# BurnhamG/PyTorch-ScalableFHVAE

Hardware: AMD Instinct MI355X
Metric: segments/sec + ELBO (nats/frame), (B,20,80) fbank (higher is better)
Workload: dtype bf16

## Files before the change

### include/fhvae_hip.h

```cpp
#ifndef FHVAE_HIP_H
#define FHVAE_HIP_H

#include <stdint.h>

#ifdef __cplusplus
extern "C" {
#endif

#define FHVAE_ABI_VERSION 11

enum { FHVAE_F32 = 0, FHVAE_BF16 = 1 };

enum {
  FHVAE_OK = 0,
  FHVAE_ERR_NULL = -1,
  FHVAE_ERR_SHAPE = -2,
  FHVAE_ERR_DTYPE = -3,
  FHVAE_ERR_ALIGN = -4,
  FHVAE_ERR_LIMIT = -5
};

#define FHVAE_MAX_LAYERS 4
#define FHVAE_LSTM_SYNC_BYTES 16384

// ... 46 lines not shown
  const float* b_ih[FHVAE_MAX_LAYERS];
  const float* b_hh[FHVAE_MAX_LAYERS];
  void* hs;
  float* cs;
  void* gates;
  float* hn;
  float* hs_top_f32;
  float* pre;
  void* lp;
  void* hn_lp;
  const float* head_w_mu;
  const float* head_w_lv;
  void* head_wl;
  void* head_wt;
  int64_t head_D, head_K, head_ldt;
  int32_t* sticky_status;
} fhvae_lstm_desc;

int64_t fhvae_lstm_lp_bytes(const fhvae_lstm_desc* d);
int64_t fhvae_lstm_pre_elems(const fhvae_lstm_desc* d);
int fhvae_lstm_layout_id(const fhvae_lstm_desc* d);

int64_t fhvae_lstm_ws_below_elems(const fhvae_lstm_desc* d);
int fhvae_lstm_form(const fhvae_lstm_desc* d);
int fhvae_lstm_seq_fwd(const fhvae_lstm_desc* d, void* stream);

typedef struct fhvae_lstm_bwd_desc {
  fhvae_lstm_desc f;
  const float* d_hs_top;
  const float* d_hn;
  void* dgates;
  float* dgsum;
  float* dc;
  float* dw_ih[FHVAE_MAX_LAYERS];
  float* dw_hh[FHVAE_MAX_LAYERS];
  float* db_ih[FHVAE_MAX_LAYERS];
  float* db_hh[FHVAE_MAX_LAYERS];
  float* d_xc;
  int32_t phase;
  float* ws_below;
} fhvae_lstm_bwd_desc;

int fhvae_lstm_seq_bwd(const fhvae_lstm_bwd_desc* d, void* stream);
typedef struct fhvae_wgrad_desc {
  const void* a; int64_t lda;
  int64_t a_col0;
  const void* b; int64_t ldb;
  float* c; int64_t ldc;
  int64_t M, N, K;
} fhvae_wgrad_desc;
int fhvae_wgrad_desc_ok(const fhvae_wgrad_desc* p);
int fhvae_lstm_param_grads_multi(const fhvae_lstm_bwd_desc* const* descs, int n, const fhvae_wgrad_desc* extra, int n_extra,
                                 void* stream);
int fhvae_wgrad_bf16(const void* a, int64_t lda, const void* b, int64_t ldb, float* c, int64_t ldc, int64_t M,
                     int64_t N, int64_t K, void* stream);
int fhvae_wgrad_f32(const float* a, int64_t lda, const float* b, int64_t ldb, float* c, int64_t ldc, int64_t M, int64_t N,
                    int64_t K, void* stream);

int fhvae_proj_bf16(const void* a, int64_t lda, const void* b, int64_t ldb, const float* bias, float* c, int64_t ldc,
                    int64_t M, int64_t N, int64_t K, void* stream);

int fhvae_mu2_gather_fwd(const float* table, const int64_t* idx, int64_t idx_offset, float* mu2,
                         int64_t B, int64_t S, int64_t D, int32_t* oob_flag, void* stream);
int fhvae_mu2_gather_bwd(const float* dmu2, const int64_t* idx, int64_t idx_offset, float* dtable,
                         int64_t B, int64_t S, int64_t D, float scale, void* stream);

typedef struct fhvae_elbo_desc {
  int64_t B, T, F, D1, D2;
  const float* x;    int64_t x_sb, x_st;
  const float* x_mu; const float* x_lv; int64_t xo_sb, xo_st;
  const float* z1_mu; const float* z1_lv;
  const float* z2_mu; const float* z2_lv;
  const float* mu2;
  const int64_t* num_segs; double nsegs_scalar;
  float* lower_bound; float* log_px_z; float* neg_kld_z1; float* neg_kld_z2; float* log_pmu2;
} fhvae_elbo_desc;

int fhvae_elbo_fwd(const fhvae_elbo_desc* d, void* stream);

typedef struct fhvae_elbo_bwd_desc {
  fhvae_elbo_desc f;
  const float* g_lower_bound; const float* g_log_px_z; const float* g_neg_kld_z1;
  const float* g_neg_kld_z2; const float* g_log_pmu2;
  int32_t reference_detach;
  float* d_x_mu; float* d_x_lv;
  float* d_z1_mu; float* d_z1_lv; float* d_z2_mu; float* d_z2_lv; float* d_mu2;
  void* d_x_pair_lp; int64_t ld_pair; float* d_x_colsum;
} fhvae_elbo_bwd_desc;

int fhvae_elbo_bwd(const fhvae_elbo_bwd_desc* d, void* stream);
int64_t fhvae_elbo_colsum_rows(int64_t B);

int64_t fhvae_disc_lse_ws_bytes(int64_t B, int64_t S);
int fhvae_disc_lse_fwd(const float* q, const float* table, const int64_t* idx, int64_t row0,
                       float inv_two_var, float* row_max, float* row_sumexp, float* tgt_logit,
                       float* ce_mean, float ce_scale, void* ws, int64_t B, int64_t S, int64_t D, int dtype, void* stream);
int fhvae_shard_pack(const float* q, const int64_t* idx, float* out, int64_t B, int64_t D, void* stream);
int fhvae_shard_unpack(const float* packed, float* q, int64_t* idx, int64_t N, int64_t D, void* stream);
int fhvae_disc_merge_partials(const float* parts, float* row_max, float* row_sumexp, float* tgt_logit, int64_t W, int64_t N,
                              void* stream);
int fhvae_shard_bwd_pack(const float* dq_all, float dq_scale, const float* dmu2_local, int64_t own0, int64_t n_own, float* out,
                         int64_t N, int64_t D, void* stream);
int fhvae_shard_bwd_unpack(const float* buf, int64_t own0, int64_t n_own, float* dq_local, float* dmu2_all, int64_t N, int64_t D,
                           void* stream);
int fhvae_disc_ce_mean(const float* row_max, const float* row_sumexp, const float* tgt_logit,
                       float* ce_mean, float ce_scale, int64_t B, void* stream);
// ... 40 lines not shown
```

### pytorch-scalablefhvae_amd/csrc/lstm.hip

```cpp
#include "gemm_launch.h"
#include "lstm_cell.h"
#include "lstm_cluster.h"
#include "wgrad.h"
#include "wgrad_f32.h"
#include <algorithm>
#include <vector>
#include "trace.h"
#include <cstdlib>

namespace fh {

constexpr int kCH = 32;

struct GateRowMap {
  int H;
  __device__ __forceinline__ int64_t operator()(int n) const {
    int unit = (n >> 6) * 16 + (n & 15);
    int gate = (n & 63) >> 4;
    return unit < H ? (int64_t)gate * H + unit : -1;
  }
  __device__ __forceinline__ bool all_valid(int n0, int n) const { return ((n0 + n) >> 6) * 16 <= H; }
};

template <typename T>
// ... 693 lines not shown
  if constexpr (!kF32) {
    if (cluster_eligible(d)) {
      ClusterWeights cw = {};
      for (int l = 0; l < L; ++l) cw.w_ih[l] = op.w_ih[l], cw.w_hh[l] = op.w_hh[l], cw.w_ih_t[l] = op.w_ih_t[l], cw.w_hh_t[l] = op.w_hh_t[l];
      cw.xch = (u16*)d->lp + lp_layout(d).xch;
      return cluster_bwd(bd, cw, st);
    }
  }
  if (big_cells(B, H, d->dtype) && cell_bwd_plan_ok(bd, op)) {
    for (int64_t w = 0; w < T_ + L - 1; ++w) {
      int nj = 0;
      const BwdJobs<T> jobs = bwd_jobs<T>(bd, op, w, nj);
      double fl = 0;
      for (int j = 0; j < nj; ++j) fl += 2.0 * B * H * (jobs.job[j].seg[0].K + jobs.job[j].seg[1].K);
      const int ts = trace_begin(st, kTraceBwdCell, fl);
      const int e = launch_cell_bwd_big(jobs, nj, st);
      trace_end(st, ts);
      if (e) return e;
    }
    if (Ic > 0) return launch_cell_dgsum((const T*)bd->dgates, bd->dgsum, (int)T_, B * 4 * H, st);
    return FHVAE_OK;
  }
  for (int64_t w = 0; w < T_ + L - 1; ++w) {
    int nj = 0;
    const BwdJobs<T> jobs = bwd_jobs<T>(bd, op, w, nj);
    double fl = 0;
    for (int j = 0; j < nj; ++j) fl += 2.0 * B * H * (jobs.job[j].seg[0].K + jobs.job[j].seg[1].K);
    const int ts = trace_begin(st, kTraceBwdCell, fl);
    const int bt = B >= 16384 ? 128 : 32;
    if (bt == 128) {
      dim3 grid((unsigned)fh_cdiv(B, 128), (unsigned)fh_cdiv(H, 64), (unsigned)nj);
      hipLaunchKernelGGL((lstm_bwd_step_kernel<T, 128, 64, 4, 1, 16>), grid, dim3(kThreads), 0, st, jobs);
    } else if (bt == 64) {
      dim3 grid((unsigned)fh_cdiv(B, 64), (unsigned)fh_cdiv(H, 64), (unsigned)nj);
      hipLaunchKernelGGL((lstm_bwd_step_kernel<T, 64, 64, 2, 2, 16>), grid, dim3(kThreads), 0, st, jobs);
    } else if (B >= 1024) {
      dim3 grid((unsigned)fh_cdiv(B, 32), (unsigned)fh_cdiv(H, 32), (unsigned)nj);
      hipLaunchKernelGGL((lstm_bwd_step_kernel<T, 32, 32, 2, 2, 16>), grid, dim3(kThreads), 0, st, jobs);
    } else {
      dim3 grid((unsigned)fh_cdiv(B, 32), (unsigned)fh_cdiv(H, 32), (unsigned)nj);
      hipLaunchKernelGGL((lstm_bwd_step_kernel<T, 32, 32, 2, 2, kCH>), grid, dim3(kThreads), 0, st, jobs);
    }
    trace_end(st, ts);
    int e = fh_launch_status();
    if (e) return e;
  }
  return FHVAE_OK;
}

constexpr int64_t kWgradMinK = 1024;

template <typename T>
static int lstm_param_grads(const fhvae_lstm_bwd_desc* bd, const Ops<T>& op, hipStream_t st, std::vector<WgProblem>* wq = nullptr,
                            std::vector<GemmParams>* fq = nullptr, std::vector<WgProblem32>* wq32 = nullptr) {
  const fhvae_lstm_desc* d = &bd->f;
  const int64_t B = d->B, T_ = d->T, I = d->I, Ic = d->Ic, H = d->H;
  const int L = d->L;
  const int64_t K0 = I + Ic, G = 4 * H;
  const T* dg = (const T*)bd->dgates;
  const T* hs = (const T*)d->hs;
  GemmParams grp[2 * FHVAE_MAX_LAYERS];
  int ng = 0;
  auto wgrad_long = [&](const void* a, int64_t lda, const void* b, int64_t ldb, int64_t Kc, float* c, int64_t ldc, int64_t Ncols) {
    if (sizeof(T) == 4) {
      if (!wq32 || Kc < kWgradMinK) return false;
      WgProblem32 w = {};
      w.A = (const float*)a, w.B = (const float*)b, w.C = c;
      w.lda = lda, w.ldb = ldb, w.ldc = ldc;
      w.M = (int)G, w.N = (int)Ncols, w.K = (int)Kc;
      if (!wgrad32_eligible(w)) return false;
      wq32->push_back(w);
      return true;
    }
    if (!wq || sizeof(T) != 2 || Kc < kWgradMinK) return false;
    WgProblem w = {};
    w.A = (const u16*)a, w.B = (const u16*)b, w.C = c;
    w.lda = lda, w.ldb = ldb, w.ldc = ldc;
    w.M = (int)G, w.N = (int)Ncols, w.K = (int)Kc;
    if (!wgrad_eligible(w)) return false;
    wq->push_back(w);
    return true;
  };
  auto wgrad = [&](const void* a, int64_t lda, const void* b, int64_t ldb, int64_t Kc, float* c, int64_t ldc, int64_t Ncols) {
    GemmParams p = {};
    p.seg[0] = Seg{a, lda, 0, b, ldb, 0, (int)Kc, 0};
    p.M = (int)G;
    p.N = (int)Ncols;
    p.C = c;
    p.ldc = ldc;
    p.splitk = 0;
    p.mode = 1;
    return p;
  };
  auto flush = [&]() -> int {
    int e = FHVAE_OK;
    for (int i = 0; i < ng && !e; i += kMaxGroup) e = launch_gemm_group(grp + i, ng - i < kMaxGroup ? ng - i : kMaxGroup, d->dtype, st);
    ng = 0;
    return e;
  };
  for (int l = 0; l < L; ++l) {
    const T* dgl = dg + (int64_t)l * T_ * B * G;
    const T* hl = hs + (int64_t)l * T_ * B * H;
    int e;
    if (bd->dw_hh[l] && T_ > 1 && !wgrad_long(dgl + B * G, G, hl, H, (T_ - 1) * B, bd->dw_hh[l], H, H))
      grp[ng++] = wgrad(dgl + B * G, G, hl, H, (T_ - 1) * B, bd->dw_hh[l], H, H);
    if (bd->dw_ih[l]) {
      if (l > 0) {
        if (!wgrad_long(dgl, G, hs + (int64_t)(l - 1) * T_ * B * H, H, T_ * B, bd->dw_ih[l], H, H))
          grp[ng++] = wgrad(dgl, G, hs + (int64_t)(l - 1) * T_ * B * H, H, T_ * B, bd->dw_ih[l], H, H);
      } else {
        if (I > 0 && !wgrad_long(dgl, G, op.x, I, T_ * B, bd->dw_ih[0], K0, I))
          grp[ng++] = wgrad(dgl, G, op.x, I, T_ * B, bd->dw_ih[0], K0, I);
        if (Ic > 0) {
          GemmParams p = wgrad(bd->dgsum, G, d->xc, Ic, B, bd->dw_ih[0] + I, K0, Ic);
          if (fq) {
            fq->push_back(p);
          } else {
            e = launch_gemm(p, FHVAE_F32, st);
            if (e) return e;
          }
        }
      }
    }
    if (!(sizeof(T) == 2 && cluster_eligible(d))) {
      if (l == 0 && Ic > 0 && bd->dgsum)
        e = launch_colsum(bd->dgsum, FHVAE_F32, G, bd->db_ih[l], bd->db_hh[l], B, G, st);
      else
        e = launch_colsum(dgl, d->dtype, G, bd->db_ih[l], bd->db_hh[l], T_ * B, G, st);
      if (e) return e;
    }
  }
  return flush();
}

static int lstm_dxc(const fhvae_lstm_bwd_desc* bd, hipStream_t st, bool zeroed = false) {
  const fhvae_lstm_desc* d = &bd->f;
  if (!bd->d_xc || d->Ic <= 0) return FHVAE_OK;
  const int64_t G = 4 * d->H, K0 = d->I + d->Ic;
  GemmParams p = {};
  p.seg[0] = Seg{bd->dgsum, G, 1, d->w_ih[0] + d->I, K0, 0, (int)G, 0};
  p.M = (int)d->B;
  p.N = (int)d->Ic;
  p.C = bd->d_xc;
  p.ldc = d->Ic;
  const int64_t tiles = fh_cdiv(d->B, 64) * fh_cdiv(d->Ic, 64);
  if (tiles <= 64 && G >= 512) {
    const int64_t n = d->B * d->Ic;
    if (!zeroed) hipLaunchKernelGGL(zero_f32_kernel, dim3((unsigned)fh_cdiv(n, 1024)), dim3(256), 0, st, bd->d_xc, n);
    p.mode = 2;
    int64_t sk = 256 / tiles;
    while (sk > 1 && G / sk < 128) sk >>= 1;
    p.splitk = (int)(sk < 4 ? 4 : sk > 16 ? 16 : sk);
  } else {
    p.splitk = 1;
  }
  return launch_gemm(p, FHVAE_F32, st);
}

extern "C" int fhvae_lstm_seq_bwd(const fhvae_lstm_bwd_desc* bd, void* stream) {
  FH_CHECK_PTR(bd);
  const fhvae_lstm_desc* d = &bd->f;
  int e = check_desc(d);
  if (e) return e;
  FH_CHECK_PTR(bd->dgates);
  FH_CHECK_PTR(bd->dc);
  if (d->Ic > 0) FH_CHECK_PTR(bd->dgsum);
  if (bd->phase < 0 || bd->phase > 2) return FHVAE_ERR_SHAPE;
  const bool rec = bd->phase != 2, par = bd->phase != 1;
  if (rec && !bd->d_hs_top && !bd->d_hn) return FHVAE_ERR_NULL;
  hipStream_t st = (hipStream_t)stream;
  if (d->dtype == FHVAE_F32) {
    Ops<float> op = ops_f32(d);
    if (rec) {
      e = lstm_bwd_impl<float>(bd, op, st);
      if (e) return e;
      e = lstm_dxc(bd, st);
      if (e) return e;
    }
    if (!par) return FHVAE_OK;
    std::vector<WgProblem32> wq32;
    e = lstm_param_grads<float>(bd, op, st, nullptr, nullptr, getenv("FHVAE_NO_WGRAD") ? nullptr : &wq32);
    if (e) return e;
    return launch_wgrad32(wq32.data(), (int)wq32.size(), st);
  }
  Ops<u16> op = ops_bf16(d);
  if (rec) {
    e = lstm_bwd_impl<u16>(bd, op, st);
    if (e) return e;
    e = lstm_dxc(bd, st, cluster_eligible(d) && cluster_bwd_zeroes_dxc(d));
    if (e) return e;
  }
  if (!par) return FHVAE_OK;
  std::vector<WgProblem> wq;
  e = lstm_param_grads<u16>(bd, op, st, getenv("FHVAE_NO_WGRAD") ? nullptr : &wq);
  if (e) return e;
  return launch_wgrad(wq.data(), (int)wq.size(), st);
}

static bool wg_from_desc(const fhvae_wgrad_desc* x, WgProblem& p) {
  if (!x || x->M <= 0 || x->N <= 0 || x->K <= 0 || x->M > INT32_MAX || x->N > INT32_MAX || x->K > INT32_MAX || x->a_col0 < 0 ||
      x->a_col0 > INT32_MAX)
    return false;
  p = WgProblem{};
  p.A = (const u16*)x->a, p.B = (const u16*)x->b, p.C = x->c;
  p.lda = x->lda, p.ldb = x->ldb, p.ldc = x->ldc;
  p.M = (int)x->M, p.N = (int)x->N, p.K = (int)x->K;
  p.a_col0 = (int)x->a_col0;
  return wgrad_eligible(p) && x->ldc >= x->N;
}

extern "C" int fhvae_wgrad_desc_ok(const fhvae_wgrad_desc* x) {
  WgProblem p;
  return wg_from_desc(x, p) ? 1 : 0;
}

extern "C" int fhvae_lstm_param_grads_multi(const fhvae_lstm_bwd_desc* const* bds, int n, const fhvae_wgrad_desc* extra, int n_extra,
                                            void* stream) {
  if (n < 0 || n_extra < 0) return FHVAE_ERR_SHAPE;
  if (n > 0) FH_CHECK_PTR(bds);
  if (n_extra > 0) FH_CHECK_PTR(extra);
  hipStream_t st = (hipStream_t)stream;
  std::vector<WgProblem> wq;
  for (int i = 0; i < n_extra; ++i) {
    WgProblem p;
    if (!wg_from_desc(extra + i, p)) return FHVAE_ERR_ALIGN;
    wq.push_back(p);
  }
  std::vector<GemmParams> fq;
  std::vector<WgProblem32> wq32;
  const bool use_wq = !getenv("FHVAE_NO_WGRAD");
  for (int i = 0; i < n; ++i) {
    const fhvae_lstm_bwd_desc* bd = bds[i];
    FH_CHECK_PTR(bd);
    const fhvae_lstm_desc* d = &bd->f;
    int e = check_desc(d);
    if (e) return e;
    FH_CHECK_PTR(bd->dgates);
    if (d->Ic > 0) FH_CHECK_PTR(bd->dgsum);
    if (d->dtype == FHVAE_F32) {
      e = lstm_param_grads<float>(bd, ops_f32(d), st, nullptr, nullptr, use_wq ? &wq32 : nullptr);
    } else {
      e = lstm_param_grads<u16>(bd, ops_bf16(d), st, use_wq ? &wq : nullptr, &fq);
    }
    if (e) return e;
  }
  for (size_t i = 0; i < fq.size();) {
    size_t j = i;
    while (j < fq.size() && j - i < (size_t)kMaxGroup) {
      bool dup = false;
      for (size_t k = i; k < j; ++k) dup = dup || fq[k].C == fq[j].C;
      if (dup) break;
      ++j;
    }
    const int e = launch_gemm_group(fq.data() + i, (int)(j - i), FHVAE_F32, st);
    if (e) return e;
    i = j;
  }
  {
    const int e = launch_wgrad32(wq32.data(), (int)wq32.size(), st);
    if (e) return e;
  }
  return launch_wgrad(wq.data(), (int)wq.size(), st);
}
```

### pytorch-scalablefhvae_amd/csrc/wgrad.h

```cpp
#pragma once
#include "common.h"

namespace fh {

struct WgProblem {
  const u16* A;
  const u16* B;
  float* C;
  int64_t lda, ldb, ldc;
  int M, N, K;
  int m_tiles, n_tiles, splitk, ksteps_per;
  int shared_c;
  int a_col0;
};

constexpr int kMaxWgProblems = 16;
struct WgGroup {
  int n;
  int base[kMaxWgProblems + 1];
  WgProblem p[kMaxWgProblems];
};

bool wgrad_eligible(const WgProblem& p);
int launch_wgrad(const WgProblem* ps, int n, hipStream_t st);

}
```

### pytorch-scalablefhvae_amd/csrc/wgrad.hip

```cpp
#include "wgrad.h"

#include <algorithm>
#include <cstdlib>

#include "gemm_core.h"

namespace fh {

constexpr int kWgThreads = 512;
constexpr int kWgBM = 256, kWgBK = 64;

template <int W>
struct WgImg {
  static constexpr int RB = W * 2;
  static constexpr int BYTES = kWgBK * RB;
  static constexpr int CPR = RB / 16;
  static constexpr int RPI = 1024 / RB;
  static constexpr int NI = BYTES / 1024 / 8;
};

typedef void __attribute__((address_space(3))) * lds_void_p;

template <int W>
__device__ __forceinline__ void wg_dma_offsets(unsigned (&voff)[WgImg<W>::NI], unsigned ld_bytes, int wave, int lane) {
  using I = WgImg<W>;
#pragma unroll
  for (int q = 0; q < I::NI; ++q) {
    const int row = (wave * I::NI + q) * I::RPI + lane / I::CPR;
    const int pc = lane % I::CPR;
    const int c = ((((pc >> 1) ^ (row & 7)) << 1) | (pc & 1));
    voff[q] = (unsigned)row * ld_bytes + (unsigned)c * 16u;
  }
}

template <int W>
__device__ __forceinline__ void wg_issue(char* stage, __amdgpu_buffer_rsrc_t rs, const unsigned (&voff)[WgImg<W>::NI], unsigned kbase,
                                         int wave) {
  using I = WgImg<W>;
#pragma unroll
  for (int q = 0; q < I::NI; ++q)
    __builtin_amdgcn_raw_ptr_buffer_load_lds(rs, (lds_void_p)(stage + (wave * I::NI + q) * 1024), 16, voff[q] + kbase, 0, 0, 0);
}

template <int RB>
__device__ __forceinline__ bf16x8 wg_frag(const char* img, int off, int j) {
  typedef s16x4 __attribute__((address_space(3))) * lds_p;
  const char* a0 = img + off + j * 32 * RB;
  union {
    struct {
      s16x4 lo, hi;
    } s;
    bf16x8 v;
  } u;
  u.s.lo = __builtin_amdgcn_ds_read_tr16_b64_v4i16((lds_p)(a0));
  u.s.hi = __builtin_amdgcn_ds_read_tr16_b64_v4i16((lds_p)(a0 + 16 * RB));
  return u.v;
}

template <int BN>
__global__ __launch_bounds__(kWgThreads) void wgrad_kernel(WgGroup g) {
  using IA = WgImg<kWgBM>;
  using IB = WgImg<BN>;
  constexpr int STAGE = IA::BYTES + IB::BYTES;
  constexpr int TM = 8, TN = BN / 64;
  constexpr int NLOAD = IA::NI + IB::NI;
  __shared__ __attribute__((aligned(1024))) char stage0[STAGE];
  __shared__ __attribute__((aligned(1024))) char stage1[STAGE];

  int wg = blockIdx.x;
  {
    const int nb = gridDim.x;
    if (nb >= 16) {
      const int q = nb >> 3, r = nb & 7, xcd = wg & 7;
      wg = (xcd < r ? xcd * (q + 1) : r * (q + 1) + (xcd - r) * q) + (wg >> 3);
    }
  }
  int pi = 0;
  while (pi + 1 < g.n && wg >= g.base[pi + 1]) ++pi;
  const WgProblem& p = g.p[pi];
  const int local = wg - g.base[pi];
  const int mt = local % p.m_tiles, nt = (local / p.m_tiles) % p.n_tiles, sp = local / (p.m_tiles * p.n_tiles);
  const int ks_total = (p.K + kWgBK - 1) / kWgBK;
  const int ks0 = sp * p.ksteps_per, ks1 = min(ks_total, ks0 + p.ksteps_per);
  if (ks0 >= ks1) return;
  const int m0 = mt * kWgBM, n0 = nt * BN;

  const int tid = threadIdx.x, lane = tid & 63, wave = tid >> 6;
  const int wm = wave >> 2, wn = wave & 3;
  const int gq = lane >> 4, i = lane & 15;

  const unsigned lda_b = (unsigned)p.lda * 2u, ldb_b = (unsigned)p.ldb * 2u;
  const __amdgpu_buffer_rsrc_t rsa =
      __builtin_amdgcn_make_buffer_rsrc(const_cast<u16*>(p.A + m0), 0, (int)(((int64_t)p.K * p.lda - p.a_col0 - m0) * 2), 0x00020000);
  const __amdgpu_buffer_rsrc_t rsb =
      __builtin_amdgcn_make_buffer_rsrc(const_cast<u16*>(p.B + n0), 0, (int)(((int64_t)p.K * p.ldb - n0) * 2), 0x00020000);
  unsigned va[IA::NI], vb[IB::NI];
  wg_dma_offsets<kWgBM>(va, lda_b, wave, lane);
  wg_dma_offsets<BN>(vb, ldb_b, wave, lane);
  auto a_step = [&](int ks) -> unsigned { return (unsigned)(ks * kWgBK) * lda_b; };

  const int kr = 4 * gq + (i >> 2), x = kr & 7;
  int offa[TM], offb[TN];
#pragma unroll
  for (int tm = 0; tm < TM; ++tm) offa[tm] = kr * IA::RB + ((((wm * 8 + tm)) ^ x) << 5) + 8 * (i & 3);
#pragma unroll
  for (int tn = 0; tn < TN; ++tn) offb[tn] = kr * IB::RB + ((((wn * TN + tn)) ^ x) << 5) + 8 * (i & 3);

  f32x4 acc[TM][TN];
#pragma unroll
  for (int tm = 0; tm < TM; ++tm)
#pragma unroll
    for (int tn = 0; tn < TN; ++tn) acc[tm][tn] = f32x4{0.f, 0.f, 0.f, 0.f};

  constexpr unsigned kOob = 0x40000000u;
  auto issue = [&](char* st, int ks) {
    const bool in = ks < ks1;
    wg_issue<kWgBM>(st, rsa, va, in ? a_step(ks) : kOob, wave);
    wg_issue<BN>(st + IA::BYTES, rsb, vb, in ? (unsigned)(ks * kWgBK) * ldb_b : kOob, wave);
  };
  auto compute = [&](const char* As, char* nxt, int ks_next) {
    const char* Bs = As + IA::BYTES;
#pragma unroll
    for (int j = 0; j < kWgBK / 32; ++j) {
      bf16x8 a[TM], b[TN];
#pragma unroll
      for (int tn = 0; tn < TN; ++tn) b[tn] = wg_frag<IB::RB>(Bs, offb[tn], j);
#pragma unroll
      for (int tm = 0; tm < TM; ++tm) a[tm] = wg_frag<IA::RB>(As, offa[tm], j);
      {
        const bool in = ks_next < ks1;
        if (j == 0)
          wg_issue<kWgBM>(nxt, rsa, va, in ? a_step(ks_next) : kOob, wave);
        else
          wg_issue<BN>(nxt + IA::BYTES, rsb, vb, in ? (unsigned)(ks_next * kWgBK) * ldb_b : kOob, wave);
      }
      __builtin_amdgcn_s_setprio(1);
#pragma unroll
      for (int tm = 0; tm < TM; ++tm)
#pragma unroll
        for (int tn = 0; tn < TN; ++tn) acc[tm][tn] = __builtin_amdgcn_mfma_f32_16x16x32_bf16(a[tm], b[tn], acc[tm][tn], 0, 0, 0);
      __builtin_amdgcn_s_setprio(0);
    }
  };
  auto step = [&](const char* cur, char* nxt, int ks_next) {
    asm volatile("s_waitcnt vmcnt(0)" ::: "memory");
    __builtin_amdgcn_s_barrier();
    compute(cur, nxt, ks_next);
    __builtin_amdgcn_s_barrier();
  };
  issue(stage0, ks0);
  for (int ks = ks0; ks < ks1; ks += 2) {
    step(stage0, stage1, ks + 1);
    step(stage1, stage0, ks + 2);
  }
  asm volatile("s_waitcnt vmcnt(0)" ::: "memory");

#pragma unroll
  for (int tm = 0; tm < TM; ++tm)
#pragma unroll
    for (int tn = 0; tn < TN; ++tn) {
      const int n = n0 + wn * (BN / 4) + tn * 16 + i;
#pragma unroll
      for (int r = 0; r < 4; ++r) {
        const int m = m0 + wm * 128 + tm * 16 + 4 * gq + r;
        if (m < p.M && n < p.N) {
          float* c = p.C + (int64_t)m * p.ldc + n;
          if (p.splitk == 1 && !p.shared_c)
            *c += acc[tm][tn][r];
          else
            atomicAdd(c, acc[tm][tn][r]);
        }
      }
    }
}

template __global__ void wgrad_kernel<256>(WgGroup);
template __global__ void wgrad_kernel<128>(WgGroup);

bool wgrad_eligible(const WgProblem& p) {
  if (p.M <= 0 || p.N <= 0 || p.K <= 0 || !p.A || !p.B || !p.C) return false;
  if ((((uintptr_t)p.A) | ((uintptr_t)p.B)) & 15) return false;
  if ((p.lda % 8) || (p.ldb % 8) || p.lda < p.a_col0 + p.M || p.ldb < p.N || p.a_col0 < 0) return false;
  if ((int64_t)p.K * p.lda * 2 >= (1LL << 30) || (int64_t)p.K * p.ldb * 2 >= (1LL << 30)) return false;
  return true;
}

template <int BN>
static int launch_class(const WgProblem* ps, const int* which, int n, hipStream_t st) {
  for (int at = 0; at < n; at += kMaxWgProblems) {
    const int cnt = n - at < kMaxWgProblems ? n - at : kMaxWgProblems;
    int64_t tiles = 0;
    for (int k = 0; k < cnt; ++k) {
      const WgProblem& p = ps[which[at + k]];
      tiles += fh_cdiv(p.M, kWgBM) * fh_cdiv(p.N, BN);
    }
    int64_t ks_max = 1;
    for (int k = 0; k < cnt; ++k) ks_max = std::max<int64_t>(ks_max, fh_cdiv(ps[which[at + k]].K, kWgBK));
    const double t_step = 2.0 * kWgBM * BN * kWgBK / (1.0e15 / 256), tile_bytes = 4.0 * kWgBM * BN;
    int64_t sk = 1;
    double best = 1e30;
    for (int64_t c = 1; c <= 64 && c * 2 <= ks_max; ++c) {
      const double waves = (double)fh_cdiv(tiles * c, 256), steps = (double)fh_cdiv(ks_max, c) + 2.0;
      const double t = waves * steps * t_step + (c > 1 ? tiles * c * tile_bytes / 1.3e12 : 0.0);
      if (t < best) best = t, sk = c;
    }
    WgGroup g = {};
    g.n = cnt;
    for (int k = 0; k < cnt; ++k) {
      WgProblem p = ps[which[at + k]];
      p.m_tiles = (int)fh_cdiv(p.M, kWgBM);
      p.n_tiles = (int)fh_cdiv(p.N, BN);
      const int64_t ks_total = fh_cdiv(p.K, kWgBK);
      int64_t s = sk;
      if (s > ks_total / 2) s = ks_total / 2;
      if (s < 1) s = 1;
      p.ksteps_per = (int)fh_cdiv(ks_total, s);
      p.splitk = (int)fh_cdiv(ks_total, p.ksteps_per);
      g.p[k] = p;
      g.base[k + 1] = g.base[k] + p.m_tiles * p.n_tiles * p.splitk;
    }
    for (int a = 0; a < cnt; ++a)
      for (int b = 0; b < cnt; ++b)
        if (a != b && g.p[a].C == g.p[b].C) g.p[a].shared_c = 1;
    const dim3 grid((unsigned)g.base[cnt]), block(kWgThreads);
    hipLaunchKernelGGL((wgrad_kernel<BN>), grid, block, 0, st, g);
    const int e = fh_launch_status();
    if (e) return e;
  }
  return FHVAE_OK;
}

int launch_wgrad(const WgProblem* ps, int n, hipStream_t st) {
  if (n <= 0) return FHVAE_OK;
  int wide[256], narrow[256], nw = 0, nn = 0;
  if (n > 256) return FHVAE_ERR_LIMIT;
  for (int k = 0; k < n; ++k) {
    if (!wgrad_eligible(ps[k])) return FHVAE_ERR_ALIGN;
    if (ps[k].N > 128)
      wide[nw++] = k;
    else
      narrow[nn++] = k;
  }
  int e = launch_class<256>(ps, wide, nw, st);
  if (e) return e;
  return launch_class<128>(ps, narrow, nn, st);
}

}

using namespace fh;

extern "C" int fhvae_wgrad_bf16(const void* a, int64_t lda, const void* b, int64_t ldb, float* c, int64_t ldc, int64_t M, int64_t N,
                                int64_t K, void* stream) {
  FH_CHECK_PTR(a);
  FH_CHECK_PTR(b);
  FH_CHECK_PTR(c);
  FH_CHECK_POS(M);
  FH_CHECK_POS(N);
  FH_CHECK_POS(K);
  FH_CHECK_I32(M);
  FH_CHECK_I32(N);
  FH_CHECK_I32(K);
  WgProblem p = {};
  p.A = (const u16*)a, p.B = (const u16*)b, p.C = c;
  p.lda = lda, p.ldb = ldb, p.ldc = ldc;
  p.M = (int)M, p.N = (int)N, p.K = (int)K;
  if (!wgrad_eligible(p)) return FHVAE_ERR_ALIGN;
  return launch_wgrad(&p, 1, (hipStream_t)stream);
}
```

### pytorch-scalablefhvae_amd/hip_binding.py

```python
from __future__ import annotations

import ctypes as C
import os
from typing import List, Optional, Sequence

import numpy as np
import torch

_HERE = os.path.dirname(os.path.abspath(__file__))
LIB_PATH = os.path.join(_HERE, "libfhvae_hip.so")

F32, BF16 = 0, 1
MAX_LAYERS = 4
ABI_VERSION = 11
PZ2_LOGVAR = np.log(0.5 ** 2).astype(np.float32)
INV_TWO_VAR = float(np.float32(1.0) / (np.float32(2.0) * np.exp(PZ2_LOGVAR)))

_vp, _i64, _i32, _f32, _f64 = C.c_void_p, C.c_int64, C.c_int32, C.c_float, C.c_double


class LstmDesc(C.Structure):
    _fields_ = [
        ("dtype", _i32), ("L", _i32),
        ("B", _i64), ("T", _i64), ("I", _i64), ("Ic", _i64), ("H", _i64),
# ... 21 lines not shown
class ElboDesc(C.Structure):
    _fields_ = [
        ("B", _i64), ("T", _i64), ("F", _i64), ("D1", _i64), ("D2", _i64),
        ("x", _vp), ("x_sb", _i64), ("x_st", _i64),
        ("x_mu", _vp), ("x_lv", _vp), ("xo_sb", _i64), ("xo_st", _i64),
        ("z1_mu", _vp), ("z1_lv", _vp), ("z2_mu", _vp), ("z2_lv", _vp), ("mu2", _vp),
        ("num_segs", _vp), ("nsegs_scalar", _f64),
        ("lower_bound", _vp), ("log_px_z", _vp), ("neg_kld_z1", _vp), ("neg_kld_z2", _vp), ("log_pmu2", _vp),
    ]


class ElboBwdDesc(C.Structure):
    _fields_ = [
        ("f", ElboDesc),
        ("g_lower_bound", _vp), ("g_log_px_z", _vp), ("g_neg_kld_z1", _vp), ("g_neg_kld_z2", _vp), ("g_log_pmu2", _vp),
        ("reference_detach", _i32),
        ("d_x_mu", _vp), ("d_x_lv", _vp), ("d_z1_mu", _vp), ("d_z1_lv", _vp), ("d_z2_mu", _vp), ("d_z2_lv", _vp),
        ("d_mu2", _vp),
        ("d_x_pair_lp", _vp), ("ld_pair", _i64), ("d_x_colsum", _vp),
    ]


class WgradDesc(C.Structure):
    _fields_ = [("a", _vp), ("lda", _i64), ("a_col0", _i64), ("b", _vp), ("ldb", _i64), ("c", _vp), ("ldc", _i64),
                ("M", _i64), ("N", _i64), ("K", _i64)]


SIGNATURES = {
    "fhvae_abi_version": (C.c_int, []),
    "fhvae_strerror": (C.c_char_p, [C.c_int]),
    "fhvae_linear_fwd": (C.c_int, [_vp, _i64, _vp, _i64, _vp, _vp, _i64, _vp, _i64, _i64, _i64, C.c_int, C.c_int, _vp]),
    "fhvae_linear_bwd": (C.c_int, [_vp, _i64, _vp, _i64, _vp, _i64, _vp, _i64, _vp, _vp, _i64, _vp, _i64, _vp, _i64, _i64,
                                   _i64, C.c_int, C.c_int, _vp]),
    "fhvae_gauss_head_reparam_fwd": (C.c_int, [_vp, _i64, _vp, _vp, _vp, _vp, _vp, _vp, _vp, _vp, _i64, _i64, _i64, C.c_int,
                                               _vp]),
    "fhvae_gauss_head_pair_fwd": (C.c_int, [_vp, _i64, _vp, _vp, _vp, _vp, _i64, _i64, _i64, _i64, _vp]),
    "fhvae_gauss_reparam_bwd": (C.c_int, [_vp, _vp, _vp, _vp, _vp, _vp, _vp, _i64, _vp]),
    "fhvae_gauss_head_bwd": (C.c_int, [_vp, _i64, _vp, _vp, _vp, _vp, _vp, _vp, _vp, _vp, _vp, _i64, _vp, _vp, _vp, _vp, _i64, _i64, _i64, _vp]),
    "fhvae_head_pair_weights": (C.c_int, [_vp, _vp, _vp, _vp, _i64, _i64, _i64, _vp]),
    "fhvae_gauss_reparam_pair_fwd": (C.c_int, [_vp, _i64, _vp, _vp, _vp, _vp, _i64, _i64, _vp]),
    "fhvae_gauss_reparam_bwd_pair": (C.c_int, [_vp, _vp, _vp, _i64, _vp, _vp, _i64, _vp, _i64, _vp, _vp, _i64, _i64, _vp]),
    "fhvae_elbo_colsum_rows": (_i64, [_i64]),
    "fhvae_gauss_head_bwd_pair": (C.c_int, [_vp, _i64, _vp, _i64, _vp, _i64, _vp, _i64, _vp, _i64, _vp, _vp, _vp, _vp, _i64, _i64, _i64, _vp]),
    "fhvae_loss_fwd": (C.c_int, [_vp, _vp, _f32, _vp, _i64, _vp, _vp]),
    "fhvae_loss_bwd": (C.c_int, [_vp, _f32, _vp, _vp, _i64, _vp]),
    "fhvae_lstm_lp_bytes": (_i64, [C.POINTER(LstmDesc)]),
    "fhvae_lstm_form": (C.c_int, [C.POINTER(LstmDesc)]),
    "fhvae_lstm_layout_id": (C.c_int, [C.POINTER(LstmDesc)]),
    "fhvae_lstm_pre_elems": (_i64, [C.POINTER(LstmDesc)]),
    "fhvae_lstm_ws_below_elems": (_i64, [C.POINTER(LstmDesc)]),
    "fhvae_lstm_seq_fwd": (C.c_int, [C.POINTER(LstmDesc), _vp]),
    "fhvae_lstm_seq_bwd": (C.c_int, [C.POINTER(LstmBwdDesc), _vp]),
    "fhvae_lstm_param_grads_multi": (C.c_int, [_vp, C.c_int, _vp, C.c_int, _vp]),
    "fhvae_wgrad_desc_ok": (C.c_int, [_vp]),
    "fhvae_wgrad_bf16": (C.c_int, [_vp, _i64, _vp, _i64, _vp, _i64, _i64, _i64, _i64, _vp]),
    "fhvae_wgrad_f32": (C.c_int, [_vp, _i64, _vp, _i64, _vp, _i64, _i64, _i64, _i64, _vp]),
    "fhvae_proj_bf16": (C.c_int, [_vp, _i64, _vp, _i64, _vp, _vp, _i64, _i64, _i64, _i64, _vp]),
    "fhvae_mu2_gather_fwd": (C.c_int, [_vp, _vp, _i64, _vp, _i64, _i64, _i64, _vp, _vp]),
    "fhvae_mu2_gather_bwd": (C.c_int, [_vp, _vp, _i64, _vp, _i64, _i64, _i64, _f32, _vp]),
    "fhvae_shard_pack": (C.c_int, [_vp, _vp, _vp, _i64, _i64, _vp]),
    "fhvae_shard_unpack": (C.c_int, [_vp, _vp, _vp, _i64, _i64, _vp]),
    "fhvae_disc_merge_partials": (C.c_int, [_vp, _vp, _vp, _vp, _i64, _i64, _vp]),
    "fhvae_shard_bwd_pack": (C.c_int, [_vp, _f32, _vp, _i64, _i64, _vp, _i64, _i64, _vp]),
    "fhvae_shard_bwd_unpack": (C.c_int, [_vp, _i64, _i64, _vp, _vp, _i64, _i64, _vp]),
    "fhvae_disc_ce_mean": (C.c_int, [_vp, _vp, _vp, _vp, _f32, _i64, _vp]),
    "fhvae_elbo_fwd": (C.c_int, [C.POINTER(ElboDesc), _vp]),
    "fhvae_elbo_bwd": (C.c_int, [C.POINTER(ElboBwdDesc), _vp]),
    "fhvae_disc_lse_ws_bytes": (_i64, [_i64, _i64]),
    "fhvae_disc_lse_bwd_ws_bytes": (_i64, [_i64, _i64, _i64]),
    "fhvae_disc_lse_fwd": (C.c_int, [_vp, _vp, _vp, _i64, _f32, _vp, _vp, _vp, _vp, _f32, _vp, _i64, _i64, _i64, C.c_int, _vp]),
    "fhvae_disc_lse_bwd": (C.c_int, [_vp, _vp, _vp, _i64, _f32, _vp, _vp, _vp, _f32, _vp, _vp, _vp, _i64, _i64, _i64, _i64, C.c_int, _vp]),
    "fhvae_adam_step": (C.c_int, [_vp, _vp, _vp, _vp, _vp, _i64, _f32, _f32, _f32, _f32, _f32, C.c_int, _vp, _vp]),
    "fhvae_segment_gather": (C.c_int, [_vp, _i64, _vp, _vp, _vp, _vp, _vp, _i64, _i64, _i64, _vp, _vp]),
    "fhvae_mu2_accumulate": (C.c_int, [_vp, _vp, _vp, _vp, _i64, _i64, _i64, _vp]),
    "fhvae_mu2_finalize": (C.c_int, [_vp, _vp, _vp, _i64, _i64, _f32, _vp]),
    "fhvae_trace_enable": (C.c_int, [C.c_int]),
    "fhvae_trace_collect": (_i64, [_vp, _vp, _vp, _i64]),
    "fhvae_to_time_major": (C.c_int, [_vp, _vp, _vp, _i64, _i64, _i64, C.c_int, _vp]),
    "fhvae_cast_bf16": (C.c_int, [_vp, _vp, _vp, _i64, _i64, _vp]),
}

_lib = None


def load_library(path: str = LIB_PATH):
    global _lib
    if _lib is not None:
        return _lib
    if not os.path.exists(path):
        raise RuntimeError(
            "libfhvae_hip.so is not built (%s). Run `python pytorch-scalablefhvae_amd/build_ext.py` "
            "(or __graft_entry__.build()). There is no CPU fallback." % path
        )
    lib = C.CDLL(path)
    for name, (res, args) in SIGNATURES.items():
        fn = getattr(lib, name)
        fn.restype = res
        fn.argtypes = args
    if lib.fhvae_abi_version() != ABI_VERSION:
        raise RuntimeError("libfhvae_hip.so ABI version mismatch")
    _lib = lib
    return lib


_SIDE = {"stream": None, "pending": False, "keep": [], "enabled": False}


LSTM_BWD_REC_HOOK = {"fn": None}


_DEFER = {"enabled": not os.environ.get("FHVAE_NO_DEFER"), "pending": [], "extra": []}


def flush_param_grads():
    pend, extra = _DEFER["pending"], _DEFER["extra"]
    if not pend and not extra:
        return
    lib = load_library()
    n, nx = len(pend), len(extra)
    arr = (C.POINTER(LstmBwdDesc) * n)(*[C.pointer(bd) for bd, _ in pend]) if n else None
    xs = (WgradDesc * nx)(*[x for x, _ in extra]) if nx else None
    with _Timed("fhvae_lstm_param_grads_multi"):
        _check(lib.fhvae_lstm_param_grads_multi(arr, n, xs, nx, _stream()), "fhvae_lstm_param_grads_multi")
    pend.clear()
    extra.clear()


def flush_param_grads_except_last():
    pend = _DEFER["pending"]
    if len(pend) <= 1:
        return
    last = pend.pop()
    flush_param_grads()
    pend.append(last)


def set_defer_param_grads(on: bool):
    flush_param_grads()
    _DEFER["enabled"] = bool(on)


def side_stream():
    if _SIDE["stream"] is None:
        _SIDE["stream"] = torch.cuda.Stream()
    return _SIDE["stream"]


def join_side_stream():
    if _SIDE["pending"]:
        torch.cuda.current_stream().wait_stream(_SIDE["stream"])
        _SIDE["pending"] = False
        _SIDE["keep"].clear()


def set_side_stream_enabled(on: bool):
    join_side_stream()
    _SIDE["enabled"] = bool(on)


class _OpTimer:

    def __init__(self):
        self.on = False
        self.pairs = []

    def enable(self):
        self.on, self.pairs = True, []

    def disable(self):
        self.on = False

    def start(self):
        e = torch.cuda.Event(enable_timing=True)
        e.record()
        return e

# ... 897 lines not shown
```

Before: 1.238 million.

## Replace split-K atomics in wgrad with slab workspace and last-block reduction

New measurement: 1.231 million, median of 6. About the same (-0.5%).

```diff
diff --git a/include/fhvae_hip.h b/include/fhvae_hip.h
--- a/include/fhvae_hip.h
+++ b/include/fhvae_hip.h
@@ -122,6 +122,10 @@
 int fhvae_wgrad_desc_ok(const fhvae_wgrad_desc* p);
 int fhvae_lstm_param_grads_multi(const fhvae_lstm_bwd_desc* const* descs, int n, const fhvae_wgrad_desc* extra, int n_extra,
                                  void* stream);
+int64_t fhvae_lstm_param_grads_ws_bytes(const fhvae_lstm_bwd_desc* const* descs, int n, const fhvae_wgrad_desc* extra,
+                                        int n_extra);
+int fhvae_lstm_param_grads_multi_ws(const fhvae_lstm_bwd_desc* const* descs, int n, const fhvae_wgrad_desc* extra, int n_extra,
+                                    void* ws, int64_t ws_bytes, void* stream);
 int fhvae_wgrad_bf16(const void* a, int64_t lda, const void* b, int64_t ldb, float* c, int64_t ldc, int64_t M,
                      int64_t N, int64_t K, void* stream);
 int fhvae_wgrad_f32(const float* a, int64_t lda, const float* b, int64_t ldb, float* c, int64_t ldc, int64_t M, int64_t N,
diff --git a/pytorch-scalablefhvae_amd/csrc/lstm.hip b/pytorch-scalablefhvae_amd/csrc/lstm.hip
--- a/pytorch-scalablefhvae_amd/csrc/lstm.hip
+++ b/pytorch-scalablefhvae_amd/csrc/lstm.hip
@@ -769,7 +769,7 @@
 
 template <typename T>
 static int lstm_param_grads(const fhvae_lstm_bwd_desc* bd, const Ops<T>& op, hipStream_t st, std::vector<WgProblem>* wq = nullptr,
-                            std::vector<GemmParams>* fq = nullptr, std::vector<WgProblem32>* wq32 = nullptr) {
+                            std::vector<GemmParams>* fq = nullptr, std::vector<WgProblem32>* wq32 = nullptr, bool dry = false) {
   const fhvae_lstm_desc* d = &bd->f;
   const int64_t B = d->B, T_ = d->T, I = d->I, Ic = d->Ic, H = d->H;
   const int L = d->L;
@@ -811,6 +811,7 @@
   };
   auto flush = [&]() -> int {
     int e = FHVAE_OK;
+    if (dry) ng = 0;
     for (int i = 0; i < ng && !e; i += kMaxGroup) e = launch_gemm_group(grp + i, ng - i < kMaxGroup ? ng - i : kMaxGroup, d->dtype, st);
     ng = 0;
     return e;
@@ -832,14 +833,14 @@
           GemmParams p = wgrad(bd->dgsum, G, d->xc, Ic, B, bd->dw_ih[0] + I, K0, Ic);
           if (fq) {
             fq->push_back(p);
-          } else {
+          } else if (!dry) {
             e = launch_gemm(p, FHVAE_F32, st);
             if (e) return e;
           }
         }
       }
     }
-    if (!(sizeof(T) == 2 && cluster_eligible(d))) {
+    if (!dry && !(sizeof(T) == 2 && cluster_eligible(d))) {
       if (l == 0 && Ic > 0 && bd->dgsum)
         e = launch_colsum(bd->dgsum, FHVAE_F32, G, bd->db_ih[l], bd->db_hh[l], B, G, st);
       else
@@ -931,13 +932,11 @@
   return wg_from_desc(x, p) ? 1 : 0;
 }
 
-extern "C" int fhvae_lstm_param_grads_multi(const fhvae_lstm_bwd_desc* const* bds, int n, const fhvae_wgrad_desc* extra, int n_extra,
-                                            void* stream) {
+static int param_grads_collect(const fhvae_lstm_bwd_desc* const* bds, int n, const fhvae_wgrad_desc* extra, int n_extra,
+                               hipStream_t st, bool dry, std::vector<WgProblem>& wq) {
   if (n < 0 || n_extra < 0) return FHVAE_ERR_SHAPE;
   if (n > 0) FH_CHECK_PTR(bds);
   if (n_extra > 0) FH_CHECK_PTR(extra);
-  hipStream_t st = (hipStream_t)stream;
-  std::vector<WgProblem> wq;
   for (int i = 0; i < n_extra; ++i) {
     WgProblem p;
     if (!wg_from_desc(extra + i, p)) return FHVAE_ERR_ALIGN;
@@ -955,12 +954,14 @@
     FH_CHECK_PTR(bd->dgates);
     if (d->Ic > 0) FH_CHECK_PTR(bd->dgsum);
     if (d->dtype == FHVAE_F32) {
+      if (dry) continue;
       e = lstm_param_grads<float>(bd, ops_f32(d), st, nullptr, nullptr, use_wq ? &wq32 : nullptr);
     } else {
-      e = lstm_param_grads<u16>(bd, ops_bf16(d), st, use_wq ? &wq : nullptr, &fq);
+      e = lstm_param_grads<u16>(bd, ops_bf16(d), st, use_wq ? &wq : nullptr, &fq, nullptr, dry);
     }
     if (e) return e;
   }
+  if (dry) return FHVAE_OK;
   for (size_t i = 0; i < fq.size();) {
     size_t j = i;
     while (j < fq.size() && j - i < (size_t)kMaxGroup) {
@@ -973,9 +974,27 @@
     if (e) return e;
     i = j;
   }
-  {
-    const int e = launch_wgrad32(wq32.data(), (int)wq32.size(), st);
-    if (e) return e;
-  }
-  return launch_wgrad(wq.data(), (int)wq.size(), st);
-}
+  return launch_wgrad32(wq32.data(), (int)wq32.size(), st);
+}
+
+extern "C" int fhvae_lstm_param_grads_multi(const fhvae_lstm_bwd_desc* const* bds, int n, const fhvae_wgrad_desc* extra, int n_extra,
+                                            void* stream) {
+  return fhvae_lstm_param_grads_multi_ws(bds, n, extra, n_extra, nullptr, 0, stream);
+}
+
+extern "C" int64_t fhvae_lstm_param_grads_ws_bytes(const fhvae_lstm_bwd_desc* const* bds, int n, const fhvae_wgrad_desc* extra,
+                                                   int n_extra) {
+  std::vector<WgProblem> wq;
+  const int e = param_grads_collect(bds, n, extra, n_extra, nullptr, true, wq);
+  if (e) return e;
+  return wgrad_workspace_bytes(wq.data(), (int)wq.size());
+}
+
+extern "C" int fhvae_lstm_param_grads_multi_ws(const fhvae_lstm_bwd_desc* const* bds, int n, const fhvae_wgrad_desc* extra,
+                                               int n_extra, void* ws, int64_t ws_bytes, void* stream) {
+  hipStream_t st = (hipStream_t)stream;
+  std::vector<WgProblem> wq;
+  const int e = param_grads_collect(bds, n, extra, n_extra, st, false, wq);
+  if (e) return e;
+  return launch_wgrad(wq.data(), (int)wq.size(), st, ws, ws_bytes);
+}
diff --git a/pytorch-scalablefhvae_amd/csrc/wgrad.h b/pytorch-scalablefhvae_amd/csrc/wgrad.h
--- a/pytorch-scalablefhvae_amd/csrc/wgrad.h
+++ b/pytorch-scalablefhvae_amd/csrc/wgrad.h
@@ -9,19 +9,25 @@
   float* C;
   int64_t lda, ldb, ldc;
   int M, N, K;
+  int bn;
   int m_tiles, n_tiles, splitk, ksteps_per;
   int shared_c;
   int a_col0;
+  int tile0;
+  int64_t slab0;
 };
 
-constexpr int kMaxWgProblems = 16;
+constexpr int kMaxWgProblems = 24;
 struct WgGroup {
   int n;
   int base[kMaxWgProblems + 1];
+  unsigned* cnt;
+  float* slab;
   WgProblem p[kMaxWgProblems];
 };
 
 bool wgrad_eligible(const WgProblem& p);
-int launch_wgrad(const WgProblem* ps, int n, hipStream_t st);
+int64_t wgrad_workspace_bytes(const WgProblem* ps, int n);
+int launch_wgrad(const WgProblem* ps, int n, hipStream_t st, void* ws = nullptr, int64_t ws_bytes = 0);
 
 }
diff --git a/pytorch-scalablefhvae_amd/csrc/wgrad.hip b/pytorch-scalablefhvae_amd/csrc/wgrad.hip
--- a/pytorch-scalablefhvae_amd/csrc/wgrad.hip
+++ b/pytorch-scalablefhvae_amd/csrc/wgrad.hip
@@ -58,27 +58,11 @@
 }
 
 template <int BN>
-__global__ __launch_bounds__(kWgThreads) void wgrad_kernel(WgGroup g) {
+__device__ __forceinline__ void wg_tile(const WgGroup& g, const WgProblem& p, int local, char* stage0, char* stage1) {
+#if defined(__HIP_DEVICE_COMPILE__)
   using IA = WgImg<kWgBM>;
   using IB = WgImg<BN>;
-  constexpr int STAGE = IA::BYTES + IB::BYTES;
   constexpr int TM = 8, TN = BN / 64;
-  constexpr int NLOAD = IA::NI + IB::NI;
-  __shared__ __attribute__((aligned(1024))) char stage0[STAGE];
-  __shared__ __attribute__((aligned(1024))) char stage1[STAGE];
-
-  int wg = blockIdx.x;
-  {
-    const int nb = gridDim.x;
-    if (nb >= 16) {
-      const int q = nb >> 3, r = nb & 7, xcd = wg & 7;
-      wg = (xcd < r ? xcd * (q + 1) : r * (q + 1) + (xcd - r) * q) + (wg >> 3);
-    }
-  }
-  int pi = 0;
-  while (pi + 1 < g.n && wg >= g.base[pi + 1]) ++pi;
-  const WgProblem& p = g.p[pi];
-  const int local = wg - g.base[pi];
   const int mt = local % p.m_tiles, nt = (local / p.m_tiles) % p.n_tiles, sp = local / (p.m_tiles * p.n_tiles);
   const int ks_total = (p.K + kWgBK - 1) / kWgBK;
   const int ks0 = sp * p.ksteps_per, ks1 = min(ks_total, ks0 + p.ksteps_per);
@@ -155,6 +139,52 @@
   }
   asm volatile("s_waitcnt vmcnt(0)" ::: "memory");
 
+  bool plain = p.splitk == 1 && !p.shared_c;
+  if (p.splitk > 1 && g.slab) {
+    const int tile = mt + p.m_tiles * nt;
+    f32x4* slabs = (f32x4*)(g.slab + p.slab0 + (int64_t)tile * p.splitk * (kWgBM * BN));
+    constexpr int kSlab4 = kWgBM * BN / 4;
+    {
+      typedef unsigned u32x4 __attribute__((ext_vector_type(4)));
+      const __amdgpu_buffer_rsrc_t rss =
+          __builtin_amdgcn_make_buffer_rsrc(slabs + (int64_t)sp * kSlab4, 0, kSlab4 * 16, 0x00020000);
+#pragma unroll
+      for (int tm = 0; tm < TM; ++tm)
+#pragma unroll
+        for (int tn = 0; tn < TN; ++tn)
+          __builtin_amdgcn_raw_buffer_store_b128(__builtin_bit_cast(u32x4, acc[tm][tn]), rss, ((tm * TN + tn) * kWgThreads + tid) * 16,
+                                                 0, 16);
+    }
+    asm volatile("s_waitcnt vmcnt(0)" ::: "memory");
+    __syncthreads();
+    int* flag = (int*)stage0;
+    if (tid == 0) {
+      unsigned* cnt = g.cnt + (int64_t)(p.tile0 + tile) * 32;
+      const unsigned t = __hip_atomic_fetch_add(cnt, 1u, __ATOMIC_RELAXED, __HIP_MEMORY_SCOPE_AGENT);
+      const int last = t == (unsigned)(p.splitk - 1);
+      if (last) {
+        __hip_atomic_store(cnt, 0u, __ATOMIC_RELAXED, __HIP_MEMORY_SCOPE_AGENT);
+        __builtin_amdgcn_fence(__ATOMIC_ACQUIRE, "agent");
+        asm volatile("s_waitcnt vmcnt(0)" ::: "memory");
+      }
+      *flag = last;
+    }
+    __syncthreads();
+    if (!*flag) return;
+#pragma unroll
+    for (int tm = 0; tm < TM; ++tm)
+#pragma unroll
+      for (int tn = 0; tn < TN; ++tn) acc[tm][tn] = slabs[(tm * TN + tn) * kWgThreads + tid];
+    for (int s = 1; s < p.splitk; ++s) {
+      const f32x4* sl = slabs + (int64_t)s * kSlab4;
+#pragma unroll
+      for (int tm = 0; tm < TM; ++tm)
+#pragma unroll
+        for (int tn = 0; tn < TN; ++tn) acc[tm][tn] += sl[(tm * TN + tn) * kWgThreads + tid];
+    }
+    plain = true;
+  }
+
 #pragma unroll
   for (int tm = 0; tm < TM; ++tm)
 #pragma unroll
@@ -165,17 +195,37 @@
         const int m = m0 + wm * 128 + tm * 16 + 4 * gq + r;
         if (m < p.M && n < p.N) {
           float* c = p.C + (int64_t)m * p.ldc + n;
-          if (p.splitk == 1 && !p.shared_c)
+          if (plain)
             *c += acc[tm][tn][r];
           else
             atomicAdd(c, acc[tm][tn][r]);
         }
       }
     }
-}
-
-template __global__ void wgrad_kernel<256>(WgGroup);
-template __global__ void wgrad_kernel<128>(WgGroup);
+#endif
+}
+
+__global__ __launch_bounds__(kWgThreads) void wgrad_kernel(WgGroup g) {
+  constexpr int STAGE = WgImg<kWgBM>::BYTES + WgImg<256>::BYTES;
+  __shared__ __attribute__((aligned(1024))) char stage0[STAGE];
+  __shared__ __attribute__((aligned(1024))) char stage1[STAGE];
+
+  int wg = blockIdx.x;
+  {
+    const int nb = gridDim.x;
+    if (nb >= 16) {
+      const int q = nb >> 3, r = nb & 7, xcd = wg & 7;
+      wg = (xcd < r ? xcd * (q + 1) : r * (q + 1) + (xcd - r) * q) + (wg >> 3);
+    }
+  }
+  int pi = 0;
+  while (pi + 1 < g.n && wg >= g.base[pi + 1]) ++pi;
+  const WgProblem& p = g.p[pi];
+  if (p.bn == 256)
+    wg_tile<256>(g, p, wg - g.base[pi], stage0, stage1);
+  else
+    wg_tile<128>(g, p, wg - g.base[pi], stage0, stage1);
+}
 
 bool wgrad_eligible(const WgProblem& p) {
   if (p.M <= 0 || p.N <= 0 || p.K <= 0 || !p.A || !p.B || !p.C) return false;
@@ -185,65 +235,130 @@
   return true;
 }
 
-template <int BN>
-static int launch_class(const WgProblem* ps, const int* which, int n, hipStream_t st) {
-  for (int at = 0; at < n; at += kMaxWgProblems) {
-    const int cnt = n - at < kMaxWgProblems ? n - at : kMaxWgProblems;
-    int64_t tiles = 0;
+constexpr int kWgCUs = 256;
+constexpr int64_t kWgCntBytes = 128;
+constexpr int64_t kWgMaxSplitTiles = 4096;
+constexpr int64_t kWgCntArea = kWgMaxSplitTiles * kWgCntBytes;
+
+static void wg_plan(WgGroup& g, const WgProblem* ps, const int* which, int cnt, bool ws) {
+  int64_t ks[kMaxWgProblems], tiles[kMaxWgProblems], unit[kMaxWgProblems], smax[kMaxWgProblems];
+  int64_t wmax = 1;
+  for (int k = 0; k < cnt; ++k) {
+    const WgProblem& p = ps[which[k]];
+    const int bn = p.N > 128 ? 256 : 128;
+    ks[k] = fh_cdiv(p.K, kWgBK);
+    tiles[k] = fh_cdiv(p.M, kWgBM) * fh_cdiv(p.N, bn);
+    unit[k] = bn / 128;
+    smax[k] = std::max<int64_t>(1, std::min<int64_t>(64, ks[k] / 2));
+    wmax = std::max(wmax, ks[k] * unit[k]);
+  }
+  const double t_half = 2.0 * kWgBM * 128 * kWgBK / (1.0e15 / kWgCUs);
+  auto split = [&](int k, int64_t W) { return std::min(smax[k], std::max<int64_t>(1, fh_cdiv(ks[k] * unit[k], W))); };
+  int64_t cands[kMaxWgProblems * 64 + 1], nc = 0;
+  cands[nc++] = wmax;
+  for (int k = 0; k < cnt; ++k)
+    for (int64_t s = 2; s <= smax[k]; ++s) cands[nc++] = fh_cdiv(ks[k], s) * unit[k];
+  int64_t best_w = wmax;
+  double best = 1e30;
+  for (int c = 0; c < nc; ++c) {
+    const int64_t W = cands[c];
+    int64_t wgs = 0, longest = 0;
+    double slab_bytes = 0, serial = 0;
     for (int k = 0; k < cnt; ++k) {
-      const WgProblem& p = ps[which[at + k]];
-      tiles += fh_cdiv(p.M, kWgBM) * fh_cdiv(p.N, BN);
-    }
-    int64_t ks_max = 1;
-    for (int k = 0; k < cnt; ++k) ks_max = std::max<int64_t>(ks_max, fh_cdiv(ps[which[at + k]].K, kWgBK));
-    const double t_step = 2.0 * kWgBM * BN * kWgBK / (1.0e15 / 256), tile_bytes = 4.0 * kWgBM * BN;
-    int64_t sk = 1;
-    double best = 1e30;
-    for (int64_t c = 1; c <= 64 && c * 2 <= ks_max; ++c) {
-      const double waves = (double)fh_cdiv(tiles * c, 256), steps = (double)fh_cdiv(ks_max, c) + 2.0;
-      const double t = waves * steps * t_step + (c > 1 ? tiles * c * tile_bytes / 1.3e12 : 0.0);
-      if (t < best) best = t, sk = c;
-    }
-    WgGroup g = {};
-    g.n = cnt;
-    for (int k = 0; k < cnt; ++k) {
-      WgProblem p = ps[which[at + k]];
-      p.m_tiles = (int)fh_cdiv(p.M, kWgBM);
-      p.n_tiles = (int)fh_cdiv(p.N, BN);
-      const int64_t ks_total = fh_cdiv(p.K, kWgBK);
-      int64_t s = sk;
-      if (s > ks_total / 2) s = ks_total / 2;
-      if (s < 1) s = 1;
-      p.ksteps_per = (int)fh_cdiv(ks_total, s);
-      p.splitk = (int)fh_cdiv(ks_total, p.ksteps_per);
-      g.p[k] = p;
-      g.base[k + 1] = g.base[k] + p.m_tiles * p.n_tiles * p.splitk;
-    }
-    for (int a = 0; a < cnt; ++a)
-      for (int b = 0; b < cnt; ++b)
-        if (a != b && g.p[a].C == g.p[b].C) g.p[a].shared_c = 1;
-    const dim3 grid((unsigned)g.base[cnt]), block(kWgThreads);
-    hipLaunchKernelGGL((wgrad_kernel<BN>), grid, block, 0, st, g);
-    const int e = fh_launch_status();
+      const int64_t s = split(k, W);
+      wgs += tiles[k] * s;
+      longest = std::max(longest, fh_cdiv(ks[k], s) * unit[k]);
+      if (s > 1) {
+        const double tile_bytes = 4.0 * kWgBM * 128 * unit[k];
+        slab_bytes += tiles[k] * s * tile_bytes;
+        serial = std::max(serial, s * tile_bytes);
+      }
+    }
+    int64_t split_tiles = 0;
+    for (int k = 0; k < cnt; ++k) split_tiles += split(k, W) > 1 ? tiles[k] : 0;
+    if (ws && split_tiles > kWgMaxSplitTiles) continue;
+    const double t = (double)fh_cdiv(wgs, kWgCUs) * (longest + 4) * t_half +
+                     (ws ? slab_bytes / 4.0e12 + serial / 100.0e9 : slab_bytes / 1.3e12);
+    if (t < best) best = t, best_w = W;
+  }
+  g = WgGroup{};
+  g.n = cnt;
+  int tile0 = 0;
+  int64_t slab0 = 0;
+  for (int k = 0; k < cnt; ++k) {
+    WgProblem p = ps[which[k]];
+    p.bn = unit[k] == 2 ? 256 : 128;
+    p.m_tiles = (int)fh_cdiv(p.M, kWgBM);
+    p.n_tiles = (int)fh_cdiv(p.N, p.bn);
+    p.ksteps_per = (int)fh_cdiv(ks[k], split(k, best_w));
+    p.splitk = (int)fh_cdiv(ks[k], p.ksteps_per);
+    p.shared_c = 0;
+    p.tile0 = tile0, p.slab0 = slab0;
+    if (p.splitk > 1) {
+      tile0 += p.m_tiles * p.n_tiles;
+      slab0 += (int64_t)p.m_tiles * p.n_tiles * p.splitk * kWgBM * p.bn;
+    }
+    g.p[k] = p;
+    g.base[k + 1] = g.base[k] + p.m_tiles * p.n_tiles * p.splitk;
+  }
+  for (int a = 0; a < cnt; ++a)
+    for (int b = 0; b < cnt; ++b)
+      if (a != b && g.p[a].C == g.p[b].C) g.p[a].shared_c = 1;
+  g.cnt = nullptr, g.slab = nullptr;
+}
+
+static int64_t wg_ws_bytes(const WgGroup& g) {
+  int64_t floats = 0;
+  for (int k = 0; k < g.n; ++k)
+    if (g.p[k].splitk > 1) floats += (int64_t)g.p[k].m_tiles * g.p[k].n_tiles * g.p[k].splitk * kWgBM * g.p[k].bn;
+  return floats ? kWgCntArea + floats * 4 : 0;
+}
+
+template <typename F>
+static int wg_batches(const WgProblem* ps, int n, bool ws, F&& fn) {
+  int which[kMaxWgProblems];
+  for (int at = 0; at < n;) {
+    int cnt = 0;
+    while (at + cnt < n && cnt < kMaxWgProblems) {
+      bool dup = false;
+      for (int k = 0; k < cnt && ws; ++k) dup = dup || ps[which[k]].C == ps[at + cnt].C;
+      if (dup) break;
+      which[cnt] = at + cnt;
+      ++cnt;
+    }
+    WgGroup g;
+    wg_plan(g, ps, which, cnt, ws);
+    const int e = fn(g);
     if (e) return e;
+    at += cnt;
   }
   return FHVAE_OK;
 }
 
-int launch_wgrad(const WgProblem* ps, int n, hipStream_t st) {
+int64_t wgrad_workspace_bytes(const WgProblem* ps, int n) {
+  int64_t need = 0;
+  wg_batches(ps, n, true, [&](const WgGroup& g) {
+    need = std::max(need, wg_ws_bytes(g));
+    return FHVAE_OK;
+  });
+  return need;
+}
+
+int launch_wgrad(const WgProblem* ps, int n, hipStream_t st, void* ws, int64_t ws_bytes) {
   if (n <= 0) return FHVAE_OK;
-  int wide[256], narrow[256], nw = 0, nn = 0;
-  if (n > 256) return FHVAE_ERR_LIMIT;
-  for (int k = 0; k < n; ++k) {
+  for (int k = 0; k < n; ++k)
     if (!wgrad_eligible(ps[k])) return FHVAE_ERR_ALIGN;
-    if (ps[k].N > 128)
-      wide[nw++] = k;
-    else
-      narrow[nn++] = k;
-  }
-  int e = launch_class<256>(ps, wide, nw, st);
-  if (e) return e;
-  return launch_class<128>(ps, narrow, nn, st);
+  if (ws && ((uintptr_t)ws & 127)) return FHVAE_ERR_ALIGN;
+  return wg_batches(ps, n, ws != nullptr, [&](WgGroup& g) {
+    const int64_t need = wg_ws_bytes(g);
+    if (ws && need) {
+      if (ws_bytes < need) return (int)FHVAE_ERR_LIMIT;
+      g.cnt = (unsigned*)ws;
+      g.slab = (float*)((char*)ws + kWgCntArea);
+    }
+    hipLaunchKernelGGL(wgrad_kernel, dim3((unsigned)g.base[g.n]), dim3(kWgThreads), 0, st, g);
+    return fh_launch_status();
+  });
 }
 
 }
diff --git a/pytorch-scalablefhvae_amd/hip_binding.py b/pytorch-scalablefhvae_amd/hip_binding.py
--- a/pytorch-scalablefhvae_amd/hip_binding.py
+++ b/pytorch-scalablefhvae_amd/hip_binding.py
@@ -97,6 +97,8 @@
     "fhvae_lstm_seq_fwd": (C.c_int, [C.POINTER(LstmDesc), _vp]),
     "fhvae_lstm_seq_bwd": (C.c_int, [C.POINTER(LstmBwdDesc), _vp]),
     "fhvae_lstm_param_grads_multi": (C.c_int, [_vp, C.c_int, _vp, C.c_int, _vp]),
+    "fhvae_lstm_param_grads_ws_bytes": (_i64, [_vp, C.c_int, _vp, C.c_int]),
+    "fhvae_lstm_param_grads_multi_ws": (C.c_int, [_vp, C.c_int, _vp, C.c_int, _vp, _i64, _vp]),
     "fhvae_wgrad_desc_ok": (C.c_int, [_vp]),
     "fhvae_wgrad_bf16": (C.c_int, [_vp, _i64, _vp, _i64, _vp, _i64, _i64, _i64, _i64, _vp]),
     "fhvae_wgrad_f32": (C.c_int, [_vp, _i64, _vp, _i64, _vp, _i64, _i64, _i64, _i64, _vp]),
@@ -155,6 +157,24 @@
 
 
 _DEFER = {"enabled": not os.environ.get("FHVAE_NO_DEFER"), "pending": [], "extra": []}
+_WGRAD_WS = {}
+
+
+def _wgrad_ws(lib, arr, n, xs, nx):
+    if os.environ.get("FHVAE_WGRAD_ATOMIC"):
+        return None, 0
+    need = lib.fhvae_lstm_param_grads_ws_bytes(arr, n, xs, nx)
+    _check(min(need, 0), "fhvae_lstm_param_grads_ws_bytes")
+    if need == 0:
+        return None, 0
+    key = (torch.cuda.current_device(), torch.cuda.current_stream().cuda_stream)
+    ws = _WGRAD_WS.get(key)
+    if ws is None or ws.numel() < need:
+        if torch.cuda.is_current_stream_capturing():
+            return None, 0
+        ws = torch.zeros(need, dtype=torch.uint8, device="cuda")
+        _WGRAD_WS[key] = ws
+    return _p(ws), ws.numel()
 
 
 def flush_param_grads():
@@ -165,8 +185,9 @@
     n, nx = len(pend), len(extra)
     arr = (C.POINTER(LstmBwdDesc) * n)(*[C.pointer(bd) for bd, _ in pend]) if n else None
     xs = (WgradDesc * nx)(*[x for x, _ in extra]) if nx else None
+    ws, ws_bytes = _wgrad_ws(lib, arr, n, xs, nx)
     with _Timed("fhvae_lstm_param_grads_multi"):
-        _check(lib.fhvae_lstm_param_grads_multi(arr, n, xs, nx, _stream()), "fhvae_lstm_param_grads_multi")
+        _check(lib.fhvae_lstm_param_grads_multi_ws(arr, n, xs, nx, ws, ws_bytes, _stream()), "fhvae_lstm_param_grads_multi")
     pend.clear()
     extra.clear()
 
```
